# CogitatorTech/vq

Measured on AMD Instinct MI355X. Metric: pq_encode_vectors_per_s, higher is better.
Workload: dtype f32 (bf16x3-split MFMA screen, exact f32 re-check)

## Files before the change

### vq_amd/csrc/k_screen_bf16.hip

```cpp
#include <cstdlib>

#include "kernels.hpp"

namespace vqhip {
namespace {

typedef float f32x4 __attribute__((ext_vector_type(4)));
typedef short bf16x8 __attribute__((ext_vector_type(8)));
typedef unsigned int u32x4 __attribute__((ext_vector_type(4)));

constexpr int kWavesPerBlock = 4;
constexpr int kBlock = kWavesPerBlock * 64;
constexpr uint64_t kPipeMinSteps = 8;

__host__ __device__ constexpr int pair_a(int p) { return p == 0 ? 0 : p == 1 ? 1 : p == 2 ? 0 : p == 3 ? 2 : p == 4 ? 1 : 0; }
__host__ __device__ constexpr int pair_x(int p) { return p == 0 ? 0 : p == 1 ? 0 : p == 2 ? 1 : p == 3 ? 0 : p == 4 ? 1 : 2; }

__host__ __device__ inline void split3(float v, uint32_t (&part)[3]) {
    uint32_t b0, b1, b2;
#if defined(__HIP_DEVICE_COMPILE__)
    b0 = __float_as_uint(v) & 0xFFFF0000u;
    const float r1 = v - __uint_as_float(b0);
    b1 = __float_as_uint(r1) & 0xFFFF0000u;
    const float r2 = r1 - __uint_as_float(b1);
// ... 281 lines not shown
        const uint32_t *base = prepA32 + ((size_t)s * (NT32 * groups) + (size_t)grp * NT32) * NMF * 4 * 64 + lane;
#pragma unroll
        for (int i = 0; i < NT32; ++i)
#pragma unroll
            for (int f = 0; f < NMF; ++f) {
                u32x4 v;
#pragma unroll
                for (int w = 0; w < 4; ++w) v[w] = base[((i * NMF + f) * 4 + w) * 64];
                a[i][f] = __builtin_bit_cast(bf16x8, v);
            }
        const uint32_t c_first = grp * NT32 * 32;
        const float *pc = prepCn + (size_t)s * cn_stride + c_first;
        for (uint32_t e = lane; e < NT32 * 32; e += 64) {
            float v = (c_first + e < cn_stride) ? pc[e] : 3.0e38f;
            if (cosine) v = (c_first + e < k_real) ? 0.0f : 3.0e38f;
            lds_cn[wave][e] = (v < 3.0e38f) ? v : 3.0e38f;
        }
    }
    const f32x4 *cnp = reinterpret_cast<const f32x4 *>(&lds_cn[wave][4 * h]);
    float pinf = __builtin_inff(), ninf = -__builtin_inff();
    uint32_t idx_mask = 0xFFFFFFC0u;
    asm volatile("" : "+s"(idx_mask));
    asm volatile("" : "+s"(pinf), "+s"(ninf));
    float cmax, tcoef;
    float mu[DPH];
    if (cosine) {
        cmax = 0.0f;
        tcoef = meta[s * 4 + 3];
        if (tcoef <= 3.0e38f)
            tcoef = (6.0f * SD + 2.5f * kBf16AssumedUlps * NMF + 200.0f) * 5.9604644775390625e-08f;
#pragma unroll
        for (int q = 0; q < DPH; ++q) mu[q] = 0.0f;
    } else {
        const float *cs = cen + (size_t)s * (SD + 4);
        cmax = cs[SD];
        tcoef = cs[SD + 1];
#pragma unroll
        for (int q = 0; q < DPH; ++q) mu[q] = cs[DPH * h + q];
    }

    const size_t col0 = (size_t)s * (PVW > 0 ? sdr : (uint32_t)SD) + (size_t)DPH * h;
    const size_t sub0 = (size_t)s * (PVW > 0 ? sdr : (uint32_t)SD);
    auto load_x = [&](uint64_t row, float (&x)[DPH]) {
        if (row >= n) row = n - 1;
        const float *ptr = X + row * d + col0;
        if constexpr (PVW > 0) {
            constexpr int VW = (PVW == 4 && DPH % 4 != 0) ? 2 : PVW;
            const float *first = X + row * d + sub0;
#pragma unroll
            for (int q = 0; q < DPH; q += VW) {
                const bool live = (uint32_t)(DPH * h + q) < sdr;
                const float *pq = live ? ptr + q : first;
                if constexpr (VW == 4) {
                    const float4 t = *reinterpret_cast<const float4 *>(pq);
                    x[q + 0] = live ? t.x : 0.0f;
                    x[q + 1] = live ? t.y : 0.0f;
                    x[q + 2] = live ? t.z : 0.0f;
                    x[q + 3] = live ? t.w : 0.0f;
                } else if constexpr (VW == 2) {
                    const float2 t = *reinterpret_cast<const float2 *>(pq);
                    x[q + 0] = live ? t.x : 0.0f;
                    x[q + 1] = live ? t.y : 0.0f;
                } else {
                    const float t = *pq;
                    x[q] = live ? t : 0.0f;
                }
            }
        } else if constexpr (DPH % 4 == 0) {
#pragma unroll
            for (int q = 0; q < DPH; q += 4) {
                const float4 t = *reinterpret_cast<const float4 *>(ptr + q);
                x[q + 0] = t.x;
                x[q + 1] = t.y;
                x[q + 2] = t.z;
                x[q + 3] = t.w;
            }
        } else {
#pragma unroll
            for (int q = 0; q < DPH; q += 2) {
                const float2 t = *reinterpret_cast<const float2 *>(ptr + q);
                x[q + 0] = t.x;
                x[q + 1] = t.y;
            }
        }
    };
    auto init_acc = [&](f32x16 &acc, int i) {
#pragma unroll
        for (int q = 0; q < 4; ++q) {
            const f32x4 c4 = cnp[(32 * i + 8 * q) / 4];
            acc[4 * q + 0] = c4[0];
            acc[4 * q + 1] = c4[1];
            acc[4 * q + 2] = c4[2];
            acc[4 * q + 3] = c4[3];
        }
    };

    float xn_[DPH];
    load_x(st0 * 32 + p, xn_);
    for (uint64_t st = st0; st < st1; ++st) {
        float x[DPH];
        float xo[ACC ? DPH : 1];
#pragma unroll
        for (int q = 0; q < DPH; ++q) {
            x[q] = xn_[q] - mu[q];
            if constexpr (ACC) xo[q] = xn_[q];
        }
        if (st + 1 < st1) load_x((st + 1) * 32 + p, xn_);

        uint32_t xp[3][DPH];
        float xs = 0.0f;
#pragma unroll
        for (int q = 0; q < DPH; ++q) {
            uint32_t parts[3];
            split3(x[q], parts);
            xp[0][q] = parts[0];
            xp[1][q] = parts[1];
            xp[2][q] = parts[2];
            xs = fmaf(x[q], x[q], xs);
        }
        bf16x8 b[NMF];
#pragma unroll
        for (int f = 0; f < NMF; ++f) {
            u32x4 v;
#pragma unroll
            for (int w = 0; w < 4; ++w) {
                uint32_t hw[2];
#pragma unroll
                for (int hh = 0; hh < 2; ++hh) {
                    const int flat = 8 * f + 2 * w + hh, pair = flat / DPH, dd = flat % DPH;
                    hw[hh] = (pair < 6) ? xp[pair_x(pair)][dd] : 0u;
                }
                v[w] = (hw[0] >> 16) | (hw[1] & 0xFFFF0000u);
            }
            b[f] = __builtin_bit_cast(bf16x8, v);
        }
#pragma unroll
        for (int f = 0; f < NMF; ++f) asm volatile("" ::"v"(b[f]));
        if constexpr (ACC) {
            __builtin_amdgcn_sched_barrier(0);
            acc_issue();
            __builtin_amdgcn_sched_barrier(0);
        }

        float q1[4] = {pinf, pinf, pinf, pinf}, q2[4] = {pinf, pinf, pinf, pinf};
        f32x16 acc[4];
        auto reduce8 = [&](const f32x16 &fin, int ifin, int g8) {
#pragma unroll
            for (int r = 0; r < 4; ++r) {
                const uint32_t ca = (uint32_t)((16 * ifin + 8 * g8 + r) & 63), cb = (uint32_t)((16 * ifin + 8 * g8 + 4 + r) & 63);
                const float pa = __uint_as_float((__float_as_uint(fin[8 * g8 + r]) & idx_mask) | ca);
                const float pb = __uint_as_float((__float_as_uint(fin[8 * g8 + 4 + r]) & idx_mask) | cb);
                const float t = __builtin_amdgcn_fmed3f(q1[r], pa, pb);
                q1[r] = __builtin_fminf(__builtin_fminf(q1[r], pa), pb);
                q2[r] = __builtin_fminf(q2[r], t);
            }
        };
        auto mfma = [&](f32x16 &accv, int ti, int f) {
            if ((ti * NMF + f + 1) * 4 <= 256)
                asm volatile("v_mfma_f32_32x32x16_bf16 %0, %1, %2, %0" : "+v"(accv) : "a"(a[ti][f]), "v"(b[f]));
            else
                asm volatile("v_mfma_f32_32x32x16_bf16 %0, %1, %2, %0" : "+v"(accv) : "v"(a[ti][f]), "v"(b[f]));
        };
        float snap[4] = {pinf, pinf, pinf, pinf};
        init_acc(acc[0], 0);
        if (NT32 > 1) init_acc(acc[1], 1);
        if (NT32 > 2) init_acc(acc[2], 2);
        asm volatile("s_nop 1");
#pragma unroll
        for (int f = 0; f < NMF; ++f)
            mfma(acc[0], 0, f);
        if (NT32 > 1) {
#pragma unroll
            for (int f = 0; f < NMF; ++f)
                mfma(acc[1], 1, f);
        } else {
            asm volatile("s_nop 7\n\ts_nop 7\n\ts_nop 7" ::: "memory");
        }
        if constexpr (ACC) {
            __builtin_amdgcn_sched_barrier(0);
            acc_commit();
            __builtin_amdgcn_sched_barrier(0);
        }
#pragma unroll
        for (int i = 0; i < NT32; ++i) {
            if (i + 3 < NT32) init_acc(acc[(i + 3) & 3], i + 3);
            if (i == 4) {
#pragma unroll
                for (int r = 0; r < 4; ++r) snap[r] = q1[r];
            }
            constexpr int kGroups = 4;
            if constexpr (NMF <= 6) {
#pragma unroll
                for (int f = 0; f < (NMF > kGroups ? NMF : kGroups); ++f) {
                    if (i + 2 < NT32 && f < NMF) mfma(acc[(i + 2) & 3], (i + 2 < NT32) ? i + 2 : 0, f);
                    if (f < kGroups && (f & 1)) reduce8(acc[i & 3], i, f >> 1);
                    __builtin_amdgcn_sched_barrier(0);
                }
            } else {
#pragma unroll
                for (int f = 0; f < NMF; ++f) {
                    if (i + 2 < NT32) mfma(acc[(i + 2) & 3], (i + 2 < NT32) ? i + 2 : 0, f);
#pragma unroll
                    for (int g8 = 0; g8 < kGroups / 2; ++g8)
                        if (f == ((g8 + 1) * NMF + kGroups / 2 - 1) / (kGroups / 2) - 1) reduce8(acc[i & 3], i, g8);
                    __builtin_amdgcn_sched_barrier(0);
                }
            }
            if (i + 2 >= NT32 && i + 1 < NT32) asm volatile("s_nop 7\n\ts_nop 7" ::: "memory");
        }

        auto merge2 = [&](float a1, float a2, uint32_t ai, float b1, float b2, uint32_t bi, float &o1, float &o2,
                          uint32_t &oi) {
            const float hi = __builtin_amdgcn_fmed3f(a1, b1, pinf);
            const float lo2 = __builtin_amdgcn_fmed3f(a2, b2, ninf);
            o2 = __builtin_amdgcn_fmed3f(hi, lo2, ninf);
            const bool tb = b1 < a1;
            o1 = tb ? b1 : a1;
            oi = tb ? bi : ai;
        };
        float u1, u2, w1, w2, m1, m2;
        uint32_t ui, wi, vidx;
        uint32_t vi[4];
#pragma unroll
        for (int r = 0; r < 4; ++r)
            vi[r] = (__float_as_uint(q1[r]) & 63u) + ((NT32 > 4 && q1[r] < snap[r]) ? 64u : 0u);
        merge2(q1[0], q2[0], vi[0], q1[1], q2[1], vi[1], u1, u2, ui);
        merge2(q1[2], q2[2], vi[2], q1[3], q2[3], vi[3], w1, w2, wi);
        merge2(u1, u2, ui, w1, w2, wi, m1, m2, vidx);
        uint32_t j = ((vidx >> 4) << 5) + (vidx & 3u) + (((vidx >> 2) & 3u) << 3) + 4 * h + grp * NT32 * 32;
        {
            const auto r1 = __builtin_amdgcn_permlane32_swap(__float_as_uint(m1), __float_as_uint(m1), false, false);
            const auto r2 = __builtin_amdgcn_permlane32_swap(__float_as_uint(m2), __float_as_uint(m2), false, false);
            const auto rj = __builtin_amdgcn_permlane32_swap(j, j, false, false);
            const auto rx = __builtin_amdgcn_permlane32_swap(__float_as_uint(xs), __float_as_uint(xs), false, false);
            const float a1 = __uint_as_float(r1[0]), b1 = __uint_as_float(r1[1]);
            const float a2 = __uint_as_float(r2[0]), b2 = __uint_as_float(r2[1]);
            xs = __uint_as_float(rx[0]) + __uint_as_float(rx[1]);
            const float hi = __builtin_amdgcn_fmed3f(a1, b1, pinf);
            const float lo2 = __builtin_amdgcn_fmed3f(a2, b2, ninf);
            m2 = __builtin_amdgcn_fmed3f(lo2, hi, ninf);
            const bool take = (b1 < a1) || (b1 == a1 && rj[1] < rj[0]);
            j = take ? rj[1] : rj[0];
            m1 = take ? b1 : a1;
        }
        if constexpr (G != 1) {
            const uint64_t prow = st * 32 + p;
            if (h == 0 && prow < n)
                part[((size_t)s * groups + grp) * n + prow] =
                    make_uint4(__float_as_uint(m1), __float_as_uint(m2), j, __float_as_uint(xs));
            continue;
        }
        const float xnorm = __builtin_sqrtf(xs) * 1.000001f;
        const float xn = xnorm + cmax;
        const float bnd = cosine ? xnorm : xn * xn;
        const float T = tcoef * bnd + 1e-35f * xn + 1e-37f;
        const float gap = m2 - m1;
        bool proven = (gap > T) && (fabsf(m1) <= 3.0e38f) && (T <= 3.0e38f);
        if (cosine) proven = proven && (m1 < -T) && (xnorm > 4e-10f);
        const uint64_t row = st * 32 + p;
        const bool writer = (h == 0) && (row < n);
        if (writer) {
            if (codes_t) codes_t[(size_t)s * codes_t_pitch + row] = (uint8_t)j;
            else codes[row * m + s] = (uint8_t)j;
        }
        const bool recheck = writer && !proven;
        const unsigned long long mask = __ballot(recheck);
        if (mask != 0ull) {
            if (recheck) {
                const uint32_t rank = (uint32_t)__popcll(mask & ((1ull << lane) - 1ull));
                wl_rows[(size_t)s * wl_stride + seg_first + seg_count + rank] = (uint32_t)row;
            }
            seg_count += (uint32_t)__popcll(mask);
        }
        if constexpr (ACC) {
            pend_mine = proven && (row < n);
            pend_j = j;
#pragma unroll
            for (int q = 0; q < DPH; ++q) pend_x[q] = xo[q];
            if (pend_mine && h == 0) {
                pend_before = cnts[j];
                pend_seq = atomicAdd(&cnts[j], 1u);
            }
        }
    }
    if constexpr (ACC) {
        acc_issue();
        acc_commit();
    }
    write_partial();
    if (G == 1 && lane == 0) {
        uint32_t *sg = wl_seg + ((size_t)s * n_seg + chunk) * 2;
        sg[0] = seg_first;
        sg[1] = seg_count;
    }
}

__host__ __device__ constexpr uint32_t x32p_acc_plane_bytes(int nt32) { return (uint32_t)nt32 * 32u * 8u; }
__host__ __device__ constexpr uint32_t x32p_acc_bytes_per_wave(int sd, int nt32) {
    return (uint32_t)sd * x32p_acc_plane_bytes(nt32) + 64u + ((uint32_t)nt32 * 32u + 64u) * 4u;
}
__host__ __device__ constexpr int x32p_grid_cols(int sd, bool acc, int npr, int pvw) {
    if (npr == 3) return pvw == 2 ? 0 : 8;
    if (sd == 8) return acc ? 4 : 8;
    return 0;
}

template <int SD, int NT32, bool ACC = false, int NPR = 6, int PVW = 0, int NC = x32p_grid_cols(SD, ACC, NPR, PVW)>
__global__ __launch_bounds__(kBlock, x32_two_waves(SD, NT32, NPR) ? 2 : 1) void k_assign_screen_bf16_x32p(
    const float *__restrict__ X, uint64_t n, uint32_t d, uint32_t m, const uint32_t *__restrict__ prepA32,
    const float *__restrict__ prepCn, uint32_t cn_stride, const float *__restrict__ meta,
    const uint32_t *__restrict__ sub_list, uint32_t n_sub, uint8_t *__restrict__ codes, uint32_t *__restrict__ wl_rows,
    uint32_t *__restrict__ wl_seg, uint32_t n_seg, uint64_t wl_stride, int cosine, uint32_t k_real,
    const float *__restrict__ cen, const uint8_t *__restrict__ gate_active, const uint32_t *__restrict__ gate_halt,
    uint8_t *__restrict__ codes_t, uint64_t codes_t_pitch, float *__restrict__ acc_sums, uint32_t *__restrict__ acc_counts,
    uint32_t sdr) {
    static_assert(NT32 == 8 && (SD == 8 || SD == 16), "pipelined screen: 8 tiles, sub_dim 8 or 16");
    static_assert(NPR == 6 || (NPR == 3 && SD == 16 && !ACC), "three products: sub_dim 16, encode form");
    static_assert(PVW == 0 || NPR == 3, "padded rows: three-product form only");
    constexpr int DPH = SD / 2;
    constexpr int NMF = (NPR * DPH + 7) / 8;
    static_assert(NPR * DPH == 8 * NMF, "every MFMA carries one term pair (sub_dim 16) or two (sub_dim 8), no padding slots");
    constexpr bool kTwo = x32_two_waves(SD, NT32, NPR);
    const bool halted = gate_halt && *gate_halt;
    const uint32_t lane = threadIdx.x & 63;
    const uint32_t h = lane >> 5, p = lane & 31;
    const uint32_t wave = __builtin_amdgcn_readfirstlane(threadIdx.x >> 6);
    const uint32_t gw = blockIdx.x * kWavesPerBlock + wave;
    const uint32_t n_chunks = n_seg;
    if (gw >= n_chunks * n_sub) return;
    const uint32_t vv = gw % n_sub;
    const uint32_t s = sub_list[vv];
    const uint32_t chunk = gw / n_sub;
    uint32_t *const seg_hdr = wl_seg + ((size_t)s * n_seg + chunk) * 2;
    const uint32_t n32 = (uint32_t)n;
    const uint32_t n_steps = (n32 + 31) / 32;
    const uint32_t steps_per_chunk = (n_steps + n_chunks - 1) / n_chunks;
    const uint32_t st0 = chunk * steps_per_chunk;
    uint32_t st1 = st0 + steps_per_chunk;
    if (st1 > n_steps) st1 = n_steps;
    if (halted || (gate_active && !gate_active[s])) {
        if (lane == 0) seg_hdr[0] = 0u, seg_hdr[1] = 0u;
        return;
    }
    extern __shared__ __attribute__((aligned(16))) float acc_lds[];
    uint32_t *cnts = nullptr;
    constexpr uint32_t kPlane = x32p_acc_plane_bytes(NT32);
    char *acc_wave = nullptr;
    if constexpr (ACC) {
        acc_wave = reinterpret_cast<char *>(acc_lds) + (size_t)wave * x32p_acc_bytes_per_wave(SD, NT32);
        cnts = reinterpret_cast<uint32_t *>(acc_wave + SD * kPlane + 64);
        for (uint32_t e = lane; e < (SD * kPlane + 64) / 16; e += 64) reinterpret_cast<float4 *>(acc_wave)[e] = make_float4(0.f, 0.f, 0.f, 0.f);
        for (uint32_t e = lane; e < NT32 * 32 + 64; e += 64) cnts[e] = 0u;
    }
    auto write_partial = [&]() {
        if constexpr (ACC) {
            float *ps = acc_sums + ((size_t)chunk * n_sub + vv) * k_real * SD;
            for (uint32_t e = lane; e < k_real * SD; e += 64) {
                const uint32_t j = e / SD, t = e % SD;
                ps[e] = (float)*reinterpret_cast<const double *>(acc_wave + t * kPlane + (t >= DPH ? 64u : 0u) + j * 8u);
            }
            uint32_t *pc = acc_counts + ((size_t)chunk * n_sub + vv) * k_real;
            for (uint32_t e = lane; e < k_real; e += 64) pc[e] = cnts[e];
        }
    };
    if (st0 >= st1) {
        write_partial();
        if (lane == 0) seg_hdr[0] = 0u, seg_hdr[1] = 0u;
        return;
    }
    const uint32_t nst = st1 - st0;
    const uint32_t seg_first = st0 * 32;
    uint32_t seg_count = 0;

    __shared__ __attribute__((aligned(16))) float lds_cn[kWavesPerBlock][NT32 * 32];
    bf16x8 a[NT32][NMF];
    {
        const uint32_t *base = prepA32 + (size_t)s * NT32 * NMF * 4 * 64 + lane;
#pragma unroll
        for (int i = 0; i < NT32; ++i)
#pragma unroll
            for (int f = 0; f < NMF; ++f) {
                u32x4 v;
#pragma unroll
                for (int w = 0; w < 4; ++w) v[w] = base[((i * NMF + f) * 4 + w) * 64];
                a[i][f] = __builtin_bit_cast(bf16x8, v);
            }
        const float *pc = prepCn + (size_t)s * cn_stride;
        for (uint32_t e = lane; e < NT32 * 32; e += 64) {
            float v = (e < cn_stride) ? pc[e] : 3.0e38f;
            if (cosine) v = (e < k_real) ? 0.0f : 3.0e38f;
            lds_cn[wave][e] = (v < 3.0e38f) ? v : 3.0e38f;
        }
    }
    const f32x4 *cnp = reinterpret_cast<const f32x4 *>(&lds_cn[wave][4 * h]);
    float pinf = __builtin_inff(), ninf = -__builtin_inff();
    uint32_t idx_mask = 0xFFFFFFC0u;
    asm volatile("" : "+s"(idx_mask));
    asm volatile("" : "+s"(pinf), "+s"(ninf));
    float cmax, tcoef;
    float mu[DPH];
    if (cosine) {
        cmax = 0.0f;
        tcoef = meta[s * 4 + 3];
        if (tcoef <= 3.0e38f) tcoef = (6.0f * SD + 2.5f * kBf16AssumedUlps * NMF + 200.0f) * 5.9604644775390625e-08f;
#pragma unroll
        for (int q = 0; q < DPH; ++q) mu[q] = 0.0f;
    } else {
        const float *cs = cen + (size_t)s * (SD + 4);
        cmax = cs[SD];
        tcoef = cs[SD + (NPR == 3 ? 2 : 1)];
#pragma unroll
        for (int q = 0; q < DPH; ++q) mu[q] = cs[DPH * h + q];
    }
    f32x4 mu4[DPH / 4];
#pragma unroll
    for (int q = 0; q < DPH; ++q) mu4[q / 4][q % 4] = mu[q];
    const size_t sub0 = (size_t)s * (PVW > 0 ? sdr : (uint32_t)SD);
    const char *const x_base = reinterpret_cast<const char *>(X + sub0 + (size_t)DPH * h);
    const uint32_t x_pitch = d * 4;
    uint8_t *const code_base = codes_t ? codes_t + (size_t)s * codes_t_pitch : codes + s;
    const uint32_t code_stride = codes_t ? 1u : m;
    constexpr int kDeep = kTwo ? 1 : 2;
    f32x4 xn_[kDeep][DPH / 4];
    auto load_x = [&](uint32_t row, int buf) {
        row = row < n32 ? row : n32 - 1;
        const float *ptr = reinterpret_cast<const float *>(x_base + (uint64_t)row * x_pitch);
        if constexpr (PVW > 0) {
            const float *first = ptr - DPH * h;
#pragma unroll
            for (int q = 0; q < DPH; q += PVW) {
                const bool live = (uint32_t)(DPH * h + q) < sdr;
                const float *pq = live ? ptr + q : first;
                if constexpr (PVW == 4) {
                    const f32x4 t = *reinterpret_cast<const f32x4 *>(pq);
#pragma unroll
                    for (int e = 0; e < 4; ++e) xn_[buf][q / 4][e] = live ? t[e] : 0.0f;
                } else if constexpr (PVW == 2) {
                    const float2 t = *reinterpret_cast<const float2 *>(pq);
                    xn_[buf][q / 4][q % 4 + 0] = live ? t.x : 0.0f;
                    xn_[buf][q / 4][q % 4 + 1] = live ? t.y : 0.0f;
                } else {
                    const float t = *pq;
                    xn_[buf][q / 4][q % 4] = live ? t : 0.0f;
                }
            }
        } else {
#pragma unroll
            for (int q = 0; q < DPH / 4; ++q) xn_[buf][q] = *reinterpret_cast<const f32x4 *>(ptr + 4 * q);
        }
    };
    auto init_acc = [&](f32x16 &acc, int i) {
#pragma unroll
        for (int q = 0; q < 4; ++q) {
            const f32x4 c4 = cnp[(32 * i + 8 * q) / 4];
            acc[4 * q + 0] = c4[0];
            acc[4 * q + 1] = c4[1];
            acc[4 * q + 2] = c4[2];
            acc[4 * q + 3] = c4[3];
        }
    };
    constexpr int kCnV = kTwo ? 0 : (ACC ? 4 : 6);
    f32x16 cnr[kCnV > 0 ? kCnV : 1];
#pragma unroll
    for (int i = 0; i < kCnV; ++i) init_acc(cnr[i], i);
    auto mfma = [&](f32x16 &accv, int ti, int f, const bf16x8 &bv) {
        if (f == 0 && ti < kCnV) {
            asm volatile("v_mfma_f32_32x32x16_bf16 %0, %1, %2, %3" : "=&v"(accv) : "a"(a[ti][f]), "v"(bv), "v"(cnr[ti]));
            return;
        }
        if constexpr (kTwo) asm volatile("v_mfma_f32_32x32x16_bf16 %0, %1, %2, %0" : "+v"(accv) : "v"(a[ti][f]), "v"(bv));
        else asm volatile("v_mfma_f32_32x32x16_bf16 %0, %1, %2, %0" : "+v"(accv) : "a"(a[ti][f]), "v"(bv));
    };

    bf16x8 b[2][NMF];
    auto bsel = [](int f) { return (NPR == 3 && f == 1) ? 0 : f; };
    float q1[2][2], q2[2][2];
    float xc[DPH];
    uint32_t xp[3][DPH];
    float xsT = 0.0f, xsM = 0.0f, xsN = 0.0f;
    f32x16 acc[4];

    constexpr int kSplitPieces = 1 + DPH / 4 + NMF;
    auto split_piece = [&](int k, int nb, uint32_t next_step, bool anchor = false) {
        if (k == 0) {
#pragma unroll
            for (int q = 0; q < DPH / 4; ++q) {
                if constexpr (kTwo) {
                    f32x4 dv = xn_[nb % kDeep][q] - mu4[q];
                    asm volatile("" : "+v"(dv));
                    xc[4 * q + 0] = dv[0], xc[4 * q + 1] = dv[1], xc[4 * q + 2] = dv[2], xc[4 * q + 3] = dv[3];
                } else {
#pragma unroll
                    for (int e = 0; e < 4; ++e) {
                        xc[4 * q + e] = xn_[nb % kDeep][q][e] - mu[4 * q + e];
                        asm volatile("" ::"v"(xc[4 * q + e]));
                    }
                }
            }
            xsN = 0.0f;
            load_x(next_step * 32 + p, nb % kDeep);
            if (anchor && n32 == 0xFFFFFFFFu) {
#pragma unroll
                for (int q = 0; q < DPH / 4; ++q) asm volatile("" ::"v"(xn_[nb % kDeep][q]));
            }
        } else if (k <= DPH / 4 && NPR == 3) {
#pragma unroll
            for (int w = 2 * (k - 1); w < 2 * k; ++w) {
                const float v0 = xc[2 * w], v1 = xc[2 * w + 1];
                const uint32_t p1 = cvt_pk_bf16(v0, v1);
                const float r0 = v0 - __uint_as_float(p1 << 16), r1 = v1 - __uint_as_float(p1 & 0xFFFF0000u);
                xp[0][w] = p1;
                xp[1][w] = cvt_pk_bf16(r0, r1);
                xsN = fmaf(v0, v0, xsN);
                xsN = fmaf(v1, v1, xsN);
            }
        } else if (k <= DPH / 4) {
#pragma unroll
            for (int q = 4 * (k - 1); q < 4 * k; ++q) {
                uint32_t parts[3];
                split3(xc[q], parts);
                xp[0][q] = parts[0];
                xp[1][q] = parts[1];
                xp[2][q] = parts[2];
                xsN = fmaf(xc[q], xc[q], xsN);
            }
        } else if (NPR == 3) {
            const int f = k - 1 - DPH / 4;
            if (f != 1) {
                u32x4 v;
#pragma unroll
                for (int w = 0; w < 4; ++w) v[w] = xp[f == 0 ? 0 : 1][w];
                b[nb][f] = __builtin_bit_cast(bf16x8, v);
                asm volatile("" ::"v"(b[nb][f]));
            }
        } else {
            const int f = k - 1 - DPH / 4;
            u32x4 v;
#pragma unroll
            for (int w = 0; w < 4; ++w) {
                uint32_t hw[2];
#pragma unroll
                for (int hh = 0; hh < 2; ++hh) {
                    const int flat = 8 * f + 2 * w + hh, pair = flat / DPH, dd = flat % DPH;
                    hw[hh] = xp[pair_x(pair)][dd];
                }
                v[w] = (hw[0] >> 16) | (hw[1] & 0xFFFF0000u);
            }
            b[nb][f] = __builtin_bit_cast(bf16x8, v);
            asm volatile("" ::"v"(b[nb][f]));
        }
    };
    float ta[2];
    auto min3 = [](float x, float y, float z) { return __builtin_fminf(__builtin_fminf(x, y), z); };
    auto reduce_hg = [&](const f32x16 &fin, int ifin, int hg, int par) {
        const int g8 = hg >> 1;
        const uint32_t ca = (uint32_t)(8 * ifin + 4 * g8 + (hg & 1)), cb = ca + 2u;
#pragma unroll
        for (int c = 0; c < 2; ++c) {
            const int r = 2 * (hg & 1) + c;
            const float pa = __uint_as_float((__float_as_uint(fin[8 * g8 + r]) & idx_mask) | ca);
            const float pb = __uint_as_float((__float_as_uint(fin[8 * g8 + 4 + r]) & idx_mask) | cb);
            const float t = __builtin_amdgcn_fmed3f(q1[par][c], pa, pb);
            q1[par][c] = min3(q1[par][c], pa, pb);
            if ((hg & 1) == 0) {
                ta[c] = t;
                asm volatile("" ::"v"(q1[par][c]), "v"(ta[c]));
            } else {
                q2[par][c] = min3(q2[par][c], ta[c], t);
                asm volatile("" ::"v"(q1[par][c]), "v"(q2[par][c]));
            }
        }
    };
    static_assert(NC == 0 || ((NC == 8 || NC == 4) && NMF == 3), "grid reduce: 8 or 4 column classes, two reduce gaps per phase");
    float cm[NC > 0 ? NC : 1];
    float rq1 = 0.0f, rq2 = 0.0f;
    float p_m1 = pinf, p_m2 = pinf;
    uint32_t p_j = 0;
    auto med3 = [](float x, float y, float z) { return __builtin_amdgcn_fmed3f(x, y, z); };
    auto tagged = [&](float v, uint32_t tag) { return __uint_as_float((__float_as_uint(v) & idx_mask) | tag); };
    auto reduce_grid = [&](const f32x16 &fin, int ifin, int hf) {
        if constexpr (NC == 8) {
#pragma unroll
            for (int c = 4 * hf; c < 4 * hf + 4; ++c) {
                cm[c] = ifin == 0 ? min3(fin[c], fin[c + 8], pinf) : min3(cm[c], fin[c], fin[c + 8]);
                asm volatile("" ::"v"(cm[c]));
            }
            float r = min3(fin[8 * hf], fin[8 * hf + 1], fin[8 * hf + 2]);
            r = min3(r, fin[8 * hf + 3], fin[8 * hf + 4]);
            r = min3(r, fin[8 * hf + 5], fin[8 * hf + 6]);
            r = min3(r, fin[8 * hf + 7], pinf);
            const float pr = tagged(r, (uint32_t)(2 * ifin + hf));
            if (hf == 0) {
                ta[0] = pr;
                asm volatile("" ::"v"(ta[0]));
            } else {
                const float t = med3(ifin == 0 ? pinf : rq1, ta[0], pr);
                rq1 = min3(ifin == 0 ? pinf : rq1, ta[0], pr);
                rq2 = ifin == 0 ? t : min3(rq2, t, pinf);
                asm volatile("" ::"v"(rq1), "v"(rq2));
            }
        } else if constexpr (NC == 4) {
#pragma unroll
            for (int c = 0; c < 4; ++c) {
                cm[c] = (ifin == 0 && hf == 0) ? min3(fin[c], fin[c + 4], pinf) : min3(cm[c], fin[8 * hf + c], fin[8 * hf + 4 + c]);
                asm volatile("" ::"v"(cm[c]));
            }
            float pr[2];
#pragma unroll
            for (int w = 0; w < 2; ++w) {
                float r = min3(fin[8 * hf + 4 * w], fin[8 * hf + 4 * w + 1], fin[8 * hf + 4 * w + 2]);
                r = min3(r, fin[8 * hf + 4 * w + 3], pinf);
                pr[w] = tagged(r, (uint32_t)(4 * ifin + 2 * hf + w));
            }
            const bool fresh = ifin == 0 && hf == 0;
            const float t = med3(fresh ? pinf : rq1, pr[0], pr[1]);
            rq1 = min3(fresh ? pinf : rq1, pr[0], pr[1]);
            if (hf == 0) {
                ta[0] = t;
                asm volatile("" ::"v"(rq1), "v"(ta[0]));
            } else {
                rq2 = min3(ifin == 0 ? pinf : rq2, ta[0], t);
                asm volatile("" ::"v"(rq1), "v"(rq2));
            }
        }
    };
    const uint32_t h4 = 4 * h;
    auto fold_step = [&]() {
        if constexpr (NC > 0) {
            float pc[NC];
#pragma unroll
            for (int c = 0; c < NC; ++c) pc[c] = tagged(cm[c], (uint32_t)(8 * (c >> 2) + (c & 3)));
            float c1 = min3(pc[0], pc[1], pinf), c2 = med3(pc[0], pc[1], pinf);
            float t1 = med3(c1, pc[2], pc[3]);
            c1 = min3(c1, pc[2], pc[3]);
            if constexpr (NC == 8) {
                const float t2 = med3(c1, pc[4], pc[5]);
                c1 = min3(c1, pc[4], pc[5]);
                c2 = min3(c2, t1, t2);
                t1 = med3(c1, pc[6], pc[7]);
                c1 = min3(c1, pc[6], pc[7]);
            }
            p_m2 = min3(c2, t1, rq2);
            p_m1 = rq1;
            const uint32_t cj = (__float_as_uint(c1) & 11u) | h4;
            p_j = ((__float_as_uint(rq1) & (NC == 8 ? 15u : 31u)) << (NC == 8 ? 4 : 3)) | cj;
            asm volatile("" ::"v"(p_m1), "v"(p_m2), "v"(p_j));
        }
    };
    float t_m1 = 0.0f, t_m2 = 0.0f, t_xs = 0.0f;
    uint32_t t_j = 0;
    bool t_proven = false;
    float pend_x[ACC ? DPH : 1];
    auto acc_reload = [&](uint32_t tst) {
        if constexpr (ACC) {
            uint32_t row = tst * 32 + p;
            row = row < n32 ? row : n32 - 1;
            const float *ptr = reinterpret_cast<const float *>(x_base + (uint64_t)row * x_pitch);
#pragma unroll
            for (int q = 0; q < DPH; q += 4) {
                const float4 t = *reinterpret_cast<const float4 *>(ptr + q);
                pend_x[q + 0] = t.x;
                pend_x[q + 1] = t.y;
                pend_x[q + 2] = t.z;
                pend_x[q + 3] = t.w;
            }
        }
    };
    auto acc_add_half_row = [&](bool mine) {
        if constexpr (ACC) {
            if (mine) {
                const uint32_t a0 = (uint32_t)(uintptr_t)(acc_wave) + (DPH * kPlane + 64u) * h + t_j * 8u;
                const uint32_t ac = (uint32_t)(uintptr_t)(cnts) + (h ? (NT32 * 32u + p) * 4u : t_j * 4u);
                const uint32_t one = 1u;
#pragma unroll
                for (int q = 0; q < DPH; ++q) {
                    const double v = (double)pend_x[q];
                    asm volatile("ds_add_f64 %0, %1 offset:%2" ::"v"(a0), "v"(v), "n"(q * (int)kPlane) : "memory");
                }
                asm volatile("ds_add_u32 %0, %1" ::"v"(ac), "v"(one) : "memory");
            }
        }
    };
    float pend_xr[ACC ? SD : 1];
    auto acc_reload_pair = [&](uint32_t S) {
        if constexpr (ACC) {
            uint32_t row = (S - 1 + h) * 32 + p;
            row = row < n32 ? row : n32 - 1;
            const float *ptr = reinterpret_cast<const float *>(reinterpret_cast<const char *>(X + (size_t)s * SD) + (uint64_t)row * x_pitch);
            const float *pa = ptr + DPH * h, *pb = ptr - DPH * h;
#pragma unroll
            for (int q = 0; q < SD; q += 4) {
                const float4 t = *reinterpret_cast<const float4 *>((q < DPH ? pa : pb) + q);
                pend_xr[q + 0] = t.x;
                pend_xr[q + 1] = t.y;
                pend_xr[q + 2] = t.z;
                pend_xr[q + 3] = t.w;
            }
        }
    };
    constexpr int kAccPieces = SD / 4;
    bool upd_mine = false;
    uint32_t upd_j = 0;
    auto acc_update_begin = [&](bool mine) {
        if constexpr (ACC) upd_mine = mine, upd_j = t_j;
    };
    auto acc_update_piece = [&](int k) {
        if constexpr (ACC) {
            if (upd_mine) {
                const uint32_t base = (uint32_t)(uintptr_t)(acc_wave) + upd_j * 8u;
                if (k < kAccPieces) {
                    const uint32_t a0 = base + ((4 * k < DPH) ? (DPH * kPlane + 64u) * h : (DPH * kPlane + 64u) * (1u - h));
#pragma unroll
                    for (int q = 4 * k; q < 4 * k + 4; ++q) {
                        const double v = (double)pend_xr[q];
                        asm volatile("ds_add_f64 %0, %1 offset:%2" ::"v"(a0), "v"(v), "n"((q < DPH ? q : q - DPH) * (int)kPlane) : "memory");
                    }
                } else {
                    const uint32_t ac = (uint32_t)(uintptr_t)(cnts) + upd_j * 4u;
                    const uint32_t one = 1u;
                    asm volatile("ds_add_u32 %0, %1" ::"v"(ac), "v"(one) : "memory");
                }
            }
        }
    };
    auto tail_piece = [&](int k, int tp, uint32_t tst) {
        if (k == 0 && NC > 0) {
            t_m1 = p_m1, t_m2 = p_m2, t_j = p_j;
        } else if (k == 0) {
            const float a1 = q1[tp][0], a2 = q2[tp][0], b1 = q1[tp][1], b2 = q2[tp][1];
            const float hi = __builtin_amdgcn_fmed3f(a1, b1, pinf);
            const float lo2 = __builtin_amdgcn_fmed3f(a2, b2, ninf);
            t_m2 = __builtin_amdgcn_fmed3f(hi, lo2, ninf);
            const bool tb = b1 < a1;
            t_m1 = tb ? b1 : a1;
            const uint32_t tag = __float_as_uint(t_m1) & 63u;
            t_j = ((tag & 62u) << 2) + ((tag & 1u) << 1) + (tb ? 1u : 0u) + 4 * h;
#pragma unroll
            for (int c = 0; c < 2; ++c) q1[tp][c] = pinf, q2[tp][c] = pinf;
        } else if (k == 1) {
            const auto r1 = __builtin_amdgcn_permlane32_swap(__float_as_uint(t_m1), __float_as_uint(t_m1), false, false);
            const auto r2 = __builtin_amdgcn_permlane32_swap(__float_as_uint(t_m2), __float_as_uint(t_m2), false, false);
            const auto rj = __builtin_amdgcn_permlane32_swap(t_j, t_j, false, false);
            const auto rx = __builtin_amdgcn_permlane32_swap(__float_as_uint(xsT), __float_as_uint(xsT), false, false);
            const float a1 = __uint_as_float(r1[0]), b1 = __uint_as_float(r1[1]);
            const float a2 = __uint_as_float(r2[0]), b2 = __uint_as_float(r2[1]);
            t_xs = __uint_as_float(rx[0]) + __uint_as_float(rx[1]);
            const float hi = __builtin_amdgcn_fmed3f(a1, b1, pinf);
            const float lo2 = __builtin_amdgcn_fmed3f(a2, b2, ninf);
            t_m2 = __builtin_amdgcn_fmed3f(lo2, hi, ninf);
            const bool take = (b1 < a1) || (b1 == a1 && rj[1] < rj[0]);
            t_j = take ? rj[1] : rj[0];
            t_m1 = take ? b1 : a1;
        } else if (k == 2) {
            const float xnorm = __builtin_sqrtf(t_xs) * 1.000001f;
            const float xn = xnorm + cmax;
            const float bnd = cosine ? xnorm : xn * xn;
            const float T = tcoef * bnd + 1e-35f * xn + 1e-37f;
            const float gap = t_m2 - t_m1;
            bool proven = (gap > T) && (fabsf(t_m1) <= 3.0e38f) && (T <= 3.0e38f);
            if (cosine) proven = proven && (t_m1 < -T) && (xnorm > 4e-10f);
            t_proven = proven;
        } else {
            const bool valid = tst < st1;
            const uint32_t row = tst * 32 + p;
            const uint32_t rowc = row < n32 ? row : n32 - 1;
            if (valid) code_base[(uint64_t)rowc * code_stride] = (uint8_t)t_j;
            const bool writer = (h == 0) && (row < n32) && valid;
            const bool recheck = writer && !t_proven;
            const unsigned long long mask = __ballot(recheck);
            if (mask != 0ull) {
                if (recheck) {
                    const uint32_t rank = (uint32_t)__popcll(mask & ((1ull << lane) - 1ull));
                    wl_rows[(size_t)s * wl_stride + seg_first + seg_count + rank] = (uint32_t)row;
                }
                seg_count += (uint32_t)__popcll(mask);
            }
            acc_add_half_row(t_proven && valid && (row < n32));
        }
    };

    float held_m1 = 0.0f, held_m2 = 0.0f, held_xs = 0.0f;
    uint32_t held_j = 0;
    auto tail_hold = [&]() { held_m1 = t_m1, held_m2 = t_m2, held_j = t_j, held_xs = xsT; };
    auto tail_pair_piece = [&](int k, uint32_t S, bool first) {
        if (k == 1) {
            const auto r1 = __builtin_amdgcn_permlane32_swap(__float_as_uint(held_m1), __float_as_uint(t_m1), false, false);
            const auto r2 = __builtin_amdgcn_permlane32_swap(__float_as_uint(held_m2), __float_as_uint(t_m2), false, false);
            const auto rj = __builtin_amdgcn_permlane32_swap(held_j, t_j, false, false);
            const auto rx = __builtin_amdgcn_permlane32_swap(__float_as_uint(held_xs), __float_as_uint(xsT), false, false);
            const float a1 = __uint_as_float(r1[0]), b1 = __uint_as_float(r1[1]);
            const float a2 = __uint_as_float(r2[0]), b2 = __uint_as_float(r2[1]);
            t_xs = __uint_as_float(rx[0]) + __uint_as_float(rx[1]);
            const float hi = __builtin_amdgcn_fmed3f(a1, b1, pinf);
            const float lo2 = __builtin_amdgcn_fmed3f(a2, b2, ninf);
            t_m2 = __builtin_amdgcn_fmed3f(lo2, hi, ninf);
            const bool take = (b1 < a1) || (b1 == a1 && rj[1] < rj[0]);
            t_j = take ? rj[1] : rj[0];
            t_m1 = take ? b1 : a1;
        } else {
            const bool valid = (h != 0) || !first;
            const uint32_t row = (S - 1 + h) * 32 + p;
            uint32_t srow = row, sj = t_j;
            if (first) {
                sj = __builtin_amdgcn_permlane32_swap(t_j, t_j, false, false)[1];
                srow = S * 32 + p;
            }
            const uint32_t rowc = srow < n32 ? srow : n32 - 1;
            code_base[(uint64_t)rowc * code_stride] = (uint8_t)sj;
            const bool recheck = valid && (row < n32) && !t_proven;
            const unsigned long long mask = __ballot(recheck);
            if (mask != 0ull) {
                if (recheck) {
                    const uint32_t rank = (uint32_t)__popcll(mask & ((1ull << lane) - 1ull));
                    wl_rows[(size_t)s * wl_stride + seg_first + seg_count + rank] = (uint32_t)row;
                }
                seg_count += (uint32_t)__popcll(mask);
            }
            acc_update_begin(valid && (row < n32) && t_proven);
        }
    };

    load_x(st0 * 32 + p, 0);
    if (kDeep == 2) load_x((st0 + 1) * 32 + p, 1);
#pragma unroll
    for (int k = 0; k < kSplitPieces; ++k) split_piece(k, 0, st0 + kDeep);
    xsM = xsN;
#pragma unroll
    for (int c = 0; c < 2; ++c) q1[0][c] = q2[0][c] = q1[1][c] = q2[1][c] = pinf;
    if (0 >= kCnV) init_acc(acc[0], 0);
    if (1 >= kCnV) init_acc(acc[1], 1);
    if (2 >= kCnV) init_acc(acc[2], 2);
    asm volatile("s_nop 1");
#pragma unroll
    for (int f = 0; f < NMF; ++f) mfma(acc[0], 0, f, b[0][bsel(f)]);
#pragma unroll
    for (int f = 0; f < NMF; ++f) mfma(acc[1], 1, f, b[0][bsel(f)]);
    __builtin_amdgcn_sched_barrier(0);

#pragma clang loop unroll(full)
    for (int peel = 0; peel < 2; ++peel) {
      const bool first = peel == 0;
      for (uint32_t it0 = first ? 0u : 2u; it0 < (first ? 1u : nst); it0 += 2) {
#pragma unroll
        for (int par = 0; par < 2; ++par) {
            const uint32_t st = st0 + it0 + par;
#pragma unroll
            for (int i = 0; i < NT32; ++i) {
                if ((i + 3) % NT32 >= kCnV) init_acc(acc[(i + 3) & 3], (i + 3) % NT32);
#pragma unroll
                for (int f = 0; f < NMF; ++f) {
                    if (i + 2 < NT32) mfma(acc[(i + 2) & 3], i + 2, f, b[par][bsel(f)]);
                    else mfma(acc[(i + 2) & 3], i + 2 - NT32, f, b[par ^ 1][bsel(f)]);
                    if constexpr (NMF == 6) {
                        if (f == 0) reduce_hg(acc[i & 3], i, 0, par);
                        if (f == 1) reduce_hg(acc[i & 3], i, 1, par);
                        if (f == 3) reduce_hg(acc[i & 3], i, 2, par);
                        if (f == 4) reduce_hg(acc[i & 3], i, 3, par);
                        if (f == 2 || f == 5) {
                            const int slot = 2 * i + (f == 5);
                            if (slot == 0) {
                                if (par == 0) acc_reload_pair(st);
                                split_piece(0, par ^ 1, st + 1 + kDeep, first);
                            } else if (slot <= 4) {
                                if (par == 0) {
                                    if (slot == 1) tail_piece(0, 1, st - 1), tail_hold();
                                } else {
                                    if (slot == 1) tail_piece(0, 0, st - 1);
                                    else if (slot == 3) tail_piece(2, 0, st - 1);
                                    else tail_pair_piece(slot - 1, st - 1, first);
                                }
                            }
                            else if (slot <= 10) split_piece(slot - 4, par ^ 1, st + 1 + kDeep);
                            else if (slot == 11) split_piece(7, par ^ 1, st + 1 + kDeep), split_piece(8, par ^ 1, st + 1 + kDeep);
                            if constexpr (ACC) {
                                if (par == 1 && slot >= 5 && slot < 5 + kAccPieces) acc_update_piece(slot - 5);
                                if (par == 1 && slot == 5 + kAccPieces) acc_update_piece(kAccPieces);
                            }
                        }
                    } else {
                        if constexpr (NC > 0) {
                            if (f < 2) reduce_grid(acc[i & 3], i, f);
                        } else {
                            if (f == 0) reduce_hg(acc[i & 3], i, 0, par), reduce_hg(acc[i & 3], i, 1, par);
                            if (f == 1) reduce_hg(acc[i & 3], i, 2, par), reduce_hg(acc[i & 3], i, 3, par);
                        }
                        if (f == 2) {
                            if (i == NT32 - 1) fold_step();
                            if (i == 0) {
                                if (par == 0) acc_reload_pair(st);
                                split_piece(0, par ^ 1, st + 1 + kDeep, first);
                                tail_piece(0, par ^ 1, st - 1);
                                if (par == 0) tail_hold();
                                else tail_pair_piece(1, st - 1, first);
                            } else if (i == 1) {
                                if (par == 1) tail_piece(2, 0, st - 1), tail_pair_piece(3, st - 1, first);
                                split_piece(1, par ^ 1, st + 1 + kDeep);
                            } else if (i < kSplitPieces) {
                                split_piece(i, par ^ 1, st + 1 + kDeep);
                            }
                            if constexpr (ACC) {
                                if (par == 1 && i >= 5 && i < 5 + kAccPieces) acc_update_piece(i - 5);
                                if (par == 1 && i == 5 + kAccPieces) acc_update_piece(kAccPieces);
                            }
                        }
                    }
                    __builtin_amdgcn_sched_barrier(0);
                }
            }
            xsT = xsM;
            xsM = xsN;
        }
      }
    }
    {
        const uint32_t last = st0 + ((nst + 1) & ~1u) - 1;
        acc_reload(last);
#pragma unroll
        for (int k = 0; k < 4; ++k) tail_piece(k, 1, last);
        write_partial();
    }
    if (lane == 0) seg_hdr[0] = seg_first, seg_hdr[1] = seg_count;
}

template <int G>
__global__ __launch_bounds__(256) void k_merge_partials_x32(const uint4 *__restrict__ part, uint64_t n, uint32_t m,
                                                            uint32_t sd, const uint32_t *__restrict__ sub_list,
                                                            const float *__restrict__ cen, const float *__restrict__ meta,
                                                            int cosine, uint8_t *__restrict__ codes,
                                                            uint32_t *__restrict__ wl_rows, uint32_t *__restrict__ wl_count,
                                                            uint64_t wl_stride, uint32_t k, uint32_t groups_rt) {
    const uint32_t groups = (G > 0) ? (uint32_t)G : groups_rt;
    const uint32_t s = sub_list[blockIdx.y];
    const float *cs = cen + (size_t)s * (sd + 4);
    float cmax = cs[sd], tcoef = cs[sd + 1];
    if (cosine) {
        const float nmf = (float)((6 * (sd / 2) + 7) / 8);
        cmax = 0.0f;
        tcoef = (meta[s * 4 + 3] <= 3.0e38f) ? (6.0f * (float)sd + 2.5f * kBf16AssumedUlps * nmf + 200.0f) * 5.9604644775390625e-08f
                                             : __builtin_inff();
    }
    const uint32_t lane = threadIdx.x & 63;
    for (uint64_t row0 = (uint64_t)blockIdx.x * 256; row0 < n; row0 += (uint64_t)gridDim.x * 256) {
        const uint64_t row = row0 + threadIdx.x;
        bool recheck = false;
        if (row < n) {
            const uint4 p0 = part[((size_t)s * groups) * n + row];
            float m1 = __uint_as_float(p0.x), m2 = __uint_as_float(p0.y);
            uint32_t j = p0.z;
            const float xs = __uint_as_float(p0.w);
#pragma unroll
            for (uint32_t g = 1; g < groups; ++g) {
                const uint4 pg = part[((size_t)s * groups + g) * n + row];
                const float b1 = __uint_as_float(pg.x), b2 = __uint_as_float(pg.y);
                const float hi = fmaxf(m1, b1), lo2 = fminf(m2, b2);
                const bool take = (b1 < m1) || (b1 == m1 && pg.z < j);
                m2 = fminf(hi, lo2);
                j = take ? pg.z : j;
                m1 = take ? b1 : m1;
            }
            const float xnorm = __builtin_sqrtf(xs) * 1.000001f;
            const float xn = xnorm + cmax;
            const float T = tcoef * (cosine ? xnorm : xn * xn) + 1e-35f * xn + 1e-37f;
            bool proven = (m2 - m1 > T) && (fabsf(m1) <= 3.0e38f) && (T <= 3.0e38f);
            if (cosine) proven = proven && (m1 < -T) && (xnorm > 4e-10f);
            store_code(codes, row * m + s, j, k);
            recheck = !proven;
        }
        const unsigned long long mask = __ballot(recheck);
        if (mask != 0ull) {
            uint32_t base = 0;
            if (lane == 0) base = atomicAdd(&wl_count[s], (uint32_t)__popcll(mask));
            base = __builtin_amdgcn_readfirstlane(base);
            if (recheck) wl_rows[(size_t)s * wl_stride + base + (uint32_t)__popcll(mask & ((1ull << lane) - 1ull))] = (uint32_t)row;
        }
    }
}

template <int NCH>
__global__ __launch_bounds__(kBlock, 1) void k_assign_screen_bf16_wide(
    const float *__restrict__ X, uint64_t n, uint32_t d, const uint32_t *__restrict__ prepA, size_t chunk_stride,
    const float *__restrict__ prepCn, uint32_t cn_stride, const uint32_t *__restrict__ sub_list, uint32_t n_sub,
    int cosine, uint32_t k_real, const float *__restrict__ cen, uint4 *__restrict__ part, uint32_t groups,
    uint32_t sdr) {
    constexpr int DPH = 32, NMF = 24, SDP = 64 * NCH;
    const uint32_t lane = threadIdx.x & 63;
    const uint32_t h = lane >> 5, p = lane & 31;
    const uint32_t wave = __builtin_amdgcn_readfirstlane(threadIdx.x >> 6);
    const uint32_t gw = blockIdx.x * kWavesPerBlock + wave;
    const uint32_t total_waves = gridDim.x * kWavesPerBlock;
    const uint32_t n_virt = n_sub * groups;
    const uint32_t n_chunks = total_waves / n_virt;
    if (gw >= n_chunks * n_virt) return;
    const uint32_t vv = gw % n_virt;
    const uint32_t s = sub_list[vv / groups];
    const uint32_t grp = vv % groups;
    const uint32_t chunk = gw / n_virt;
    const uint64_t n_steps = (n + 31) / 32;
    const uint64_t steps_per_chunk = (n_steps + n_chunks - 1) / n_chunks;
    const uint64_t st0 = (uint64_t)chunk * steps_per_chunk;
    uint64_t st1 = st0 + steps_per_chunk;
    if (st1 > n_steps) st1 = n_steps;
    if (st0 >= st1) return;

    bf16x8 a[NCH][NMF];
#pragma unroll
    for (int c = 0; c < NCH; ++c) {
        const uint32_t *base = prepA + (size_t)c * chunk_stride + ((size_t)s * groups + grp) * NMF * 4 * 64 + lane;
#pragma unroll
        for (int f = 0; f < NMF; ++f) {
            u32x4 v;
#pragma unroll
            for (int w = 0; w < 4; ++w) v[w] = base[(f * 4 + w) * 64];
            a[c][f] = __builtin_bit_cast(bf16x8, v);
        }
    }
    float cnv[16];
#pragma unroll
    for (int r = 0; r < 16; ++r) {
        const uint32_t idx = grp * 32 + (r & 3) + 8 * (r >> 2) + 4 * h;
        float v = (idx < cn_stride) ? prepCn[(size_t)s * cn_stride + idx] : 3.0e38f;
        if (cosine) v = (idx < k_real) ? 0.0f : 3.0e38f;
        cnv[r] = (v < 3.0e38f) ? v : 3.0e38f;
    }
    const float *cs = cen + (size_t)s * (SDP + 4);
    const float pinf = __builtin_inff(), ninf = -__builtin_inff();
    const size_t sub0 = (size_t)s * sdr;

    for (uint64_t st = st0; st < st1; ++st) {
        uint64_t row = st * 32 + p;
        if (row >= n) row = n - 1;
        const float *xrow = X + row * d + sub0;
        f32x16 acc;
#pragma unroll
        for (int r = 0; r < 16; ++r) acc[r] = cnv[r];
        float xs = 0.0f;
#pragma unroll
        for (int c = 0; c < NCH; ++c) {
            float x[DPH];
#pragma unroll
            for (int q = 0; q < DPH; q += 4) {
                const uint32_t dim = 64 * c + DPH * h + q;
                const bool live = dim < sdr;
                const float4 t = *reinterpret_cast<const float4 *>(xrow + (live ? dim : 0u));
                float4 mu4 = make_float4(0.f, 0.f, 0.f, 0.f);
                if (!cosine) mu4 = *reinterpret_cast<const float4 *>(cs + dim);
                x[q + 0] = live ? t.x - mu4.x : 0.0f;
                x[q + 1] = live ? t.y - mu4.y : 0.0f;
                x[q + 2] = live ? t.z - mu4.z : 0.0f;
                x[q + 3] = live ? t.w - mu4.w : 0.0f;
            }
            uint32_t xp[3][DPH];
#pragma unroll
            for (int q = 0; q < DPH; ++q) {
                uint32_t parts[3];
                split3(x[q], parts);
                xp[0][q] = parts[0];
                xp[1][q] = parts[1];
                xp[2][q] = parts[2];
                xs = fmaf(x[q], x[q], xs);
            }
#pragma unroll
            for (int f = 0; f < NMF; ++f) {
                u32x4 v;
#pragma unroll
                for (int w = 0; w < 4; ++w) {
                    uint32_t hw[2];
#pragma unroll
                    for (int hh = 0; hh < 2; ++hh) {
                        const int flat = 8 * f + 2 * w + hh, pair = flat / DPH, dd = flat % DPH;
                        hw[hh] = xp[pair_x(pair)][dd];
                    }
                    v[w] = (hw[0] >> 16) | (hw[1] & 0xFFFF0000u);
                }
                acc = __builtin_amdgcn_mfma_f32_32x32x16_bf16(a[c][f], __builtin_bit_cast(bf16x8, v), acc, 0, 0, 0);
            }
        }
        float m1 = pinf, m2 = pinf;
        uint32_t ji = 0;
#pragma unroll
        for (int r = 0; r < 16; ++r) {
            const float v = acc[r];
            const uint32_t idx = (r & 3) + 8 * (r >> 2) + 4 * h;
            m2 = __builtin_amdgcn_fmed3f(m1, m2, v);
            const bool take = (v < m1) || (v == m1 && idx < ji);
            ji = take ? idx : ji;
            m1 = take ? v : m1;
        }
        uint32_t j = grp * 32 + ji;
        {
            const auto r1 = __builtin_amdgcn_permlane32_swap(__float_as_uint(m1), __float_as_uint(m1), false, false);
            const auto r2 = __builtin_amdgcn_permlane32_swap(__float_as_uint(m2), __float_as_uint(m2), false, false);
            const auto rj = __builtin_amdgcn_permlane32_swap(j, j, false, false);
            const auto rx = __builtin_amdgcn_permlane32_swap(__float_as_uint(xs), __float_as_uint(xs), false, false);
            const float a1 = __uint_as_float(r1[0]), b1 = __uint_as_float(r1[1]);
            const float a2 = __uint_as_float(r2[0]), b2 = __uint_as_float(r2[1]);
            xs = __uint_as_float(rx[0]) + __uint_as_float(rx[1]);
            const float hi = __builtin_amdgcn_fmed3f(a1, b1, pinf);
            const float lo2 = __builtin_amdgcn_fmed3f(a2, b2, ninf);
            m2 = __builtin_amdgcn_fmed3f(lo2, hi, ninf);
            const bool take = (b1 < a1) || (b1 == a1 && rj[1] < rj[0]);
            j = take ? rj[1] : rj[0];
            m1 = take ? b1 : a1;
        }
        const uint64_t prow = st * 32 + p;
        if (h == 0 && prow < n)
            part[((size_t)s * groups + grp) * n + prow] = make_uint4(__float_as_uint(m1), __float_as_uint(m2), j, __float_as_uint(xs));
    }
}

__global__ __launch_bounds__(256) void k_codes_transpose(const uint8_t *__restrict__ ct, uint64_t pitch, uint8_t *__restrict__ codes,
                                                         uint64_t n, uint32_t m, const uint32_t *__restrict__ sub_list,
                                                         uint32_t n_sub, const uint8_t *__restrict__ gate_active,
                                                         const uint32_t *__restrict__ gate_halt) {
    extern __shared__ __attribute__((aligned(16))) uint8_t tr_lds[];
    if (gate_halt && *gate_halt) return;
    const uint32_t tp = codes_transpose_pitch(m);
    uint8_t *tile = tr_lds, *act = tr_lds + 256 * tp;
    const uint64_t row0 = (uint64_t)blockIdx.x * 256;
    for (uint32_t s = threadIdx.x; s < m; s += 256) act[s] = 0;
    __syncthreads();
    for (uint32_t i = threadIdx.x; i < n_sub; i += 256) {
        const uint32_t s = sub_list[i];
        act[s] = gate_active ? gate_active[s] : (uint8_t)1;
    }
    __syncthreads();
    const uint32_t wave = threadIdx.x >> 6, lane = threadIdx.x & 63;
    for (uint32_t s0 = wave; s0 < m; s0 += 32) {
        uint32_t v[8];
#pragma unroll
        for (uint32_t u = 0; u < 8; ++u) {
            const uint32_t s = min(s0 + 4 * u, m - 1u);
            v[u] = *reinterpret_cast<const uint32_t *>(ct + (size_t)s * pitch + row0 + 4 * lane);
        }
#pragma unroll
        for (uint32_t u = 0; u < 8; ++u) {
            const uint32_t s = s0 + 4 * u;
            if (s >= m) break;
            uint32_t w = v[u];
            if (!act[s]) {
                w = 0;
#pragma unroll
                for (uint32_t i = 0; i < 4; ++i) {
                    const uint64_t r = row0 + 4 * lane + i;
                    if (r < n) w |= (uint32_t)codes[r * m + s] << (8 * i);
                }
            }
#pragma unroll
            for (uint32_t i = 0; i < 4; ++i) tile[(4 * lane + i) * tp + s] = (uint8_t)(w >> (8 * i));
        }
    }
    __syncthreads();
    const uint32_t rows_here = (uint32_t)min((uint64_t)256, n - row0), qpr = m / 4;
    uint32_t *out = reinterpret_cast<uint32_t *>(codes + row0 * m);
    for (uint32_t idx = threadIdx.x; idx < rows_here * qpr; idx += 256) {
        const uint32_t r = idx / qpr, q = idx - r * qpr;
        out[idx] = *reinterpret_cast<const uint32_t *>(tile + r * tp + 4 * q);
    }
}

template <int SD, int NT32, int G = 1, int PVW = 0, bool ACC = false>
int launch_one_x32(const CodebookView &cb, const AssignArgs &a, hipStream_t stream, uint32_t groups_rt = 0) {
    const uint32_t groups = (G > 0) ? (uint32_t)G : groups_rt;
// ... 302 lines not shown
```

Baseline: 3.973 billion.

## Use grid column-class reduction for six-product sub_dim 16 screen kernel

Switches the six-product (NMF==6) pipelined screen from per-half-group top-2 reduction to the grid column-class reduction previously used only by the three-product and sub_dim 8 paths. New NC=8 and NC=4 variants split the reduction across four MFMA gaps per phase, and a fold_step is added at slot 15. The number of centroid-norm registers held for the first MFMA drops from 6 to 5 to free VGPRs. The change alters the reduction dataflow and register pressure in the pipelined loop, which risks schedule stalls or spills.

```diff
diff --git a/vq_amd/csrc/k_screen_bf16.hip b/vq_amd/csrc/k_screen_bf16.hip
--- a/vq_amd/csrc/k_screen_bf16.hip
+++ b/vq_amd/csrc/k_screen_bf16.hip
@@ -607,7 +607,7 @@
 __host__ __device__ constexpr int x32p_grid_cols(int sd, bool acc, int npr, int pvw) {
     if (npr == 3) return pvw == 2 ? 0 : 8;
     if (sd == 8) return acc ? 4 : 8;
-    return 0;
+    return 8;
 }
 
 template <int SD, int NT32, bool ACC = false, int NPR = 6, int PVW = 0, int NC = x32p_grid_cols(SD, ACC, NPR, PVW)>
@@ -764,7 +764,7 @@
             acc[4 * q + 3] = c4[3];
         }
     };
-    constexpr int kCnV = kTwo ? 0 : (ACC ? 4 : 6);
+    constexpr int kCnV = kTwo ? 0 : (ACC ? 4 : (NC == 8 ? 5 : 6));
     f32x16 cnr[kCnV > 0 ? kCnV : 1];
 #pragma unroll
     for (int i = 0; i < kCnV; ++i) init_acc(cnr[i], i);
@@ -876,7 +876,8 @@
             }
         }
     };
-    static_assert(NC == 0 || ((NC == 8 || NC == 4) && NMF == 3), "grid reduce: 8 or 4 column classes, two reduce gaps per phase");
+    static_assert(NC == 0 || ((NC == 8 || NC == 4) && (NMF == 3 || NMF == 6)),
+                  "grid reduce: 8 or 4 column classes, two (three products) or four (six products) reduce gaps per phase");
     float cm[NC > 0 ? NC : 1];
     float rq1 = 0.0f, rq2 = 0.0f;
     float p_m1 = pinf, p_m2 = pinf;
@@ -884,7 +885,57 @@
     auto med3 = [](float x, float y, float z) { return __builtin_amdgcn_fmed3f(x, y, z); };
     auto tagged = [&](float v, uint32_t tag) { return __uint_as_float((__float_as_uint(v) & idx_mask) | tag); };
     auto reduce_grid = [&](const f32x16 &fin, int ifin, int hf) {
-        if constexpr (NC == 8) {
+        if constexpr (NC == 8 && NMF == 6) {
+#pragma unroll
+            for (int c = 2 * hf; c < 2 * hf + 2; ++c) {
+                cm[c] = ifin == 0 ? min3(fin[c], fin[c + 8], pinf) : min3(cm[c], fin[c], fin[c + 8]);
+                asm volatile("" ::"v"(cm[c]));
+            }
+            const int e0 = 8 * (hf >> 1) + 4 * (hf & 1);
+            if ((hf & 1) == 0) {
+                const float r = min3(fin[e0], fin[e0 + 1], fin[e0 + 2]);
+                ta[1] = min3(r, fin[e0 + 3], pinf);
+                asm volatile("" ::"v"(ta[1]));
+            } else {
+                float r = min3(ta[1], fin[e0], fin[e0 + 1]);
+                r = min3(r, fin[e0 + 2], fin[e0 + 3]);
+                const float pr = tagged(r, (uint32_t)(2 * ifin + (hf >> 1)));
+                if (hf == 1) {
+                    ta[0] = pr;
+                    asm volatile("" ::"v"(ta[0]));
+                } else {
+                    const float t = med3(ifin == 0 ? pinf : rq1, ta[0], pr);
+                    rq1 = min3(ifin == 0 ? pinf : rq1, ta[0], pr);
+                    rq2 = ifin == 0 ? t : min3(rq2, t, pinf);
+                    asm volatile("" ::"v"(rq1), "v"(rq2));
+                }
+            }
+        } else if constexpr (NC == 4 && NMF == 6) {
+            const int hh = hf >> 1;
+#pragma unroll
+            for (int c = 2 * (hf & 1); c < 2 * (hf & 1) + 2; ++c) {
+                cm[c] = (ifin == 0 && hh == 0) ? min3(fin[c], fin[c + 4], pinf) : min3(cm[c], fin[8 * hh + c], fin[8 * hh + 4 + c]);
+                asm volatile("" ::"v"(cm[c]));
+            }
+            float r = min3(fin[4 * hf], fin[4 * hf + 1], fin[4 * hf + 2]);
+            r = min3(r, fin[4 * hf + 3], pinf);
+            const float pr = tagged(r, (uint32_t)(4 * ifin + hf));
+            if ((hf & 1) == 0) {
+                ta[0] = pr;
+                asm volatile("" ::"v"(ta[0]));
+            } else {
+                const bool fresh = ifin == 0 && hf == 1;
+                const float t = med3(fresh ? pinf : rq1, ta[0], pr);
+                rq1 = min3(fresh ? pinf : rq1, ta[0], pr);
+                if (hf == 1) {
+                    ta[1] = t;
+                    asm volatile("" ::"v"(rq1), "v"(ta[1]));
+                } else {
+                    rq2 = min3(ifin == 0 ? pinf : rq2, ta[1], t);
+                    asm volatile("" ::"v"(rq1), "v"(rq2));
+                }
+            }
+        } else if constexpr (NC == 8) {
 #pragma unroll
             for (int c = 4 * hf; c < 4 * hf + 4; ++c) {
                 cm[c] = ifin == 0 ? min3(fin[c], fin[c + 8], pinf) : min3(cm[c], fin[c], fin[c + 8]);
@@ -1130,8 +1181,10 @@
 #pragma unroll
     for (int k = 0; k < kSplitPieces; ++k) split_piece(k, 0, st0 + kDeep);
     xsM = xsN;
-#pragma unroll
-    for (int c = 0; c < 2; ++c) q1[0][c] = q2[0][c] = q1[1][c] = q2[1][c] = pinf;
+    if constexpr (NC == 0) {
+#pragma unroll
+        for (int c = 0; c < 2; ++c) q1[0][c] = q2[0][c] = q1[1][c] = q2[1][c] = pinf;
+    }
     if (0 >= kCnV) init_acc(acc[0], 0);
     if (1 >= kCnV) init_acc(acc[1], 1);
     if (2 >= kCnV) init_acc(acc[2], 2);
@@ -1157,12 +1210,17 @@
                     if (i + 2 < NT32) mfma(acc[(i + 2) & 3], i + 2, f, b[par][bsel(f)]);
                     else mfma(acc[(i + 2) & 3], i + 2 - NT32, f, b[par ^ 1][bsel(f)]);
                     if constexpr (NMF == 6) {
-                        if (f == 0) reduce_hg(acc[i & 3], i, 0, par);
-                        if (f == 1) reduce_hg(acc[i & 3], i, 1, par);
-                        if (f == 3) reduce_hg(acc[i & 3], i, 2, par);
-                        if (f == 4) reduce_hg(acc[i & 3], i, 3, par);
+                        if constexpr (NC > 0) {
+                            if (f != 2 && f != 5) reduce_grid(acc[i & 3], i, f - (f > 2));
+                        } else {
+                            if (f == 0) reduce_hg(acc[i & 3], i, 0, par);
+                            if (f == 1) reduce_hg(acc[i & 3], i, 1, par);
+                            if (f == 3) reduce_hg(acc[i & 3], i, 2, par);
+                            if (f == 4) reduce_hg(acc[i & 3], i, 3, par);
+                        }
                         if (f == 2 || f == 5) {
                             const int slot = 2 * i + (f == 5);
+                            if (slot == 15) fold_step();
                             if (slot == 0) {
                                 if (par == 0) acc_reload_pair(st);
                                 split_piece(0, par ^ 1, st + 1 + kDeep, first);
```

Result: no change. 3.974 billion (median of 2 runs) (+0.0%).
